# weiwei-ww/ML-VAE

Measured on AMD Instinct MI355X. Metric: spectrogram frames/sec + ELBO; 80-d log-mel B=256 at 1/2/4/8 MI355X, higher is better.
Workload: dtype bf16

## Files before the change

### ml-vae_amd/csrc/lstm_wide.hip

```cpp
#include "lstm_common.h"
#include <stdlib.h>
#include <type_traits>

namespace {

constexpr int WW = 8;
constexpr int FWD_KLF = 4;
template <int TPW> constexpr int bptt_groups() { return 2; }
#ifndef NT_AUX
#define NT_AUX 2
#endif

__device__ __forceinline__ void publish(__amdgpu_buffer_rsrc_t r, unsigned byte_off,
                                        unsigned long long v, bool plain) {
  if (plain) {
    u32x2 w = {(unsigned)v, (unsigned)(v >> 32)};
    __builtin_amdgcn_raw_buffer_store_b64(w, r, byte_off, 0, 0);
  } else {
    st_granule(r, byte_off, v);
  }
}

__device__ __forceinline__ int swz(int utt, int slot) { return slot ^ (utt & 15); }

template <int TPW, int NKC, int OCC, bool DBG = false, bool AS = false, bool ZP = false, int NT = 1,
          bool W12 = false>
__global__ __launch_bounds__(W12 ? 768 : 512, W12 ? 1 : OCC) void lstm_fwd_wide_kernel(LstmArgs a) {
  static_assert(NT == 1 || (NT == 2 && AS && TPW == 1), "two N-tiles: the asymmetric TPW-1 split");
  static_assert(!W12 || (AS && TPW == 1), "12 waves: the asymmetric TPW-1 split");
  constexpr int NWV = W12 ? 12 : 8;
  constexpr int NPOLL = W12 ? 8 : 4;
  constexpr int IO0 = NWV - 4;
  constexpr int BGW = BG * NT;
  constexpr int HJ = WW * TPW * 4;
  constexpr int H = NKC * 32;
  constexpr int PL = NKC / NPOLL;
  constexpr int ROWB = H * 2;
  constexpr int HIMG = BGW * ROWB;
  constexpr int GXU = 4 * HJ + 8;
  constexpr int OUB = 4 * HJ * 2 + 2 * HJ * 4 + 16;
  constexpr int NC8 = BGW * HJ / 8;
  constexpr int KLF = ((TPW == 1 && !AS) || W12) ? 0 : FWD_KLF;
  constexpr int KR = NKC - KLF;
  constexpr int HB = 4;
  constexpr int NQ = 16 * 4 * HJ / 4;
  constexpr int QPT = NQ / 256;
  static_assert(NQ % 256 == 0, "io split");
  extern __shared__ __attribute__((aligned(16))) char smem[];
  LSTAMP_DECL;
  RTS_DECL;
  char* himg = smem;
  unsigned short* gxr = reinterpret_cast<unsigned short*>(smem + 2 * HIMG);
  char* outr = reinterpret_cast<char*>(gxr + 2 * BGW * GXU);
  bf16x8* wlds = reinterpret_cast<bf16x8*>(outr + 2 * BGW * OUB);
  unsigned* dbl = reinterpret_cast<unsigned*>(wlds + 8 * TPW * KLF * 64);
  __shared__ int abort_flag;

  const int ngroups = 2 * a.NB, gstride = (ngroups + 7) & ~7;
  const int gid = blockIdx.x % gstride, js = blockIdx.x / gstride;
  if (gid >= ngroups) return;
  const int dir = gid / a.NB, grp = gid % a.NB;
  const int T = a.T, j0 = js * HJ;
  const int tid = threadIdx.x, lane = tid & 63;
  const int nlg = (DMODE(a) & (1 << 24)) ? 2 : 1, nmask = (1 << nlg) - 1;
  const int wave = __builtin_amdgcn_readfirstlane(tid >> 6);
  const float* W = dir ? a.W1 : a.W0;
  const int bi = lane & 15, q = lane >> 4;
  bool valid[NT];
#pragma unroll
  for (int n = 0; n < NT; ++n) valid[n] = grp * BGW + 16 * n + bi < a.B;

  static_assert(!AS || TPW == 1, "asymmetric split: TPW 1 only");
  constexpr int TPP = W12 ? 1 : AS ? 2 : TPW;
  constexpr int TPI = AS ? 0 : TPW;
  static_assert(NPOLL * TPP + 4 * TPI == WW * TPW, "every tile owned once");
  auto load_w = [&](auto* wreg, int m0, int mt) {
    for (int t = 0; t < mt; ++t) {
      const int m = m0 + t;
      const float* wrow = W + (size_t)((bi & 3) * H + j0 + 4 * m + (bi >> 2)) * H;
#pragma unroll
      for (int kc = 0; kc < NKC; ++kc) {
        const f32x4 w0 = *reinterpret_cast<const f32x4*>(wrow + kc * 32 + 8 * q);
        const f32x4 w1 = *reinterpret_cast<const f32x4*>(wrow + kc * 32 + 8 * q + 4);
        bf16x8 v;
#pragma unroll
        for (int e = 0; e < 4; ++e) { v[e] = f2bf(w0[e]); v[4 + e] = f2bf(w1[e]); }
        if (kc < KR) wreg[t][kc < KR ? kc : 0] = v;
        else wlds[(m * KLF + (kc - KR)) * 64 + lane] = v;
      }
    }
  };
  __shared__ int placement;
  const bool same_xcd = group_on_one_xcd(a.xtab + gid * a.NJ, a.NJ, js, &placement) &&
                        !(DMODE(a) & 32768);
  if (tid == 0) abort_flag = 0;

  const size_t xslot = (size_t)BGW * H;
  short* xb = reinterpret_cast<short*>(a.xbuf) + (size_t)(dir * a.NB + grp) * NSLOT * xslot;
  auto xr = make_rsrc(xb, (unsigned)(NSLOT * xslot * sizeof(short)));

  const int iot = tid - 64 * IO0;
  const bool io = wave >= IO0;
  const int iow = wave - IO0;
  typedef __attribute__((address_space(3))) void* lds_ptr_t;
  unsigned short* G16 = reinterpret_cast<unsigned short*>(a.G);
  const auto rgx = make_rsrc(G16 + (size_t)grp * BGW * T * 8 * H, 0xffffffffu);
  const bool tmaj = (DMODE(a) & 1024) != 0;
  auto rowof = [&](int b_, int t_) -> size_t { return tmaj ? (size_t)t_ * a.B + b_ : (size_t)b_ * T + t_; };
  const auto rgx_abs = make_rsrc(G16, (unsigned)min((size_t)a.B * T * 8 * H * 2, (size_t)0xffffffffu));
  unsigned short* zr = gxr;
  const auto rz = make_rsrc(a.Zb, (unsigned)min((size_t)a.B * T * a.ldz * 2, (size_t)0x7fffffff));
  auto io_load = [&](int s_) {
    if (s_ >= T || (s_ > 0 && (DMODE(a) & 8192))) return;
    const int t_ = dir ? T - 1 - s_ : s_;
    if constexpr (ZP) {
      if (iow < NT) {
        const int u = iow * 16 + (lane >> 2), b = grp * BGW + u;
        const unsigned off = b < a.B ? (unsigned)((((size_t)b * T + t_) * a.ldz + 8 * (lane & 3)) * 2) : 0x80000000u;
        __builtin_amdgcn_raw_ptr_buffer_load_lds(rz, (lds_ptr_t)(zr + ((s_ & 1) * BGW + iow * 16) * 32), 16,
                                                 off, 0, 0, NT_AUX);
      }
      return;
    }
    constexpr int UPW = BGW / 4;
#pragma unroll
    for (int i = 0; i < UPW; ++i) {
      const int u = iow * UPW + i, b = grp * BGW + u;
      if (b >= a.B) continue;
      const int g = lane / (HJ / 8), uu = (lane % (HJ / 8)) * 8;
      const unsigned off = tmaj ? (unsigned)((((size_t)t_ * a.B + b) * 8 * H + dir * 4 * H + g * H + j0 + uu) * 2)
                                : (unsigned)((((size_t)u * T + t_) * 8 * H + dir * 4 * H + g * H + j0 + uu) * 2);
      const auto rs = tmaj ? rgx_abs : rgx;
      unsigned short* dst = gxr + (s_ & 1) * BGW * GXU + u * GXU;
      if (lane < HJ / 2) __builtin_amdgcn_raw_ptr_buffer_load_lds(rs, (lds_ptr_t)dst, 16, off, 0, 0, NT_AUX);
    }
  };
  auto drop_bits = [&](int s_, int c8) -> unsigned {
    const int u = c8 / (HJ / 8), uu = (c8 % (HJ / 8)) * 8;
    const int t_ = dir ? T - 1 - s_ : s_;
    const size_t o = ((size_t)(grp * BGW + u) * T + t_) * 2 * H + dir * H + j0 + uu;
    const unsigned long long k = drop_key(a.dseed);
    const unsigned long long r0 = drop_quad(k, (a.doff + o) >> 2), r1 = drop_quad(k, (a.doff + o + 4) >> 2);
    unsigned bits = 0;
#pragma unroll
    for (int e = 0; e < 4; ++e) {
      bits |= (drop_elem_scale(r0, e, a.dkeep, 1.f) != 0.f ? 1u : 0u) << e;
      bits |= (drop_elem_scale(r1, e, a.dkeep, 1.f) != 0.f ? 1u : 0u) << (4 + e);
    }
    return bits;
  };
  auto io_store = [&](int s_) {
    if (s_ < 0 || s_ >= T || (DMODE(a) & 1)) return;
    const int t_ = dir ? T - 1 - s_ : s_;
    const char* src = outr + (s_ & 1) * BGW * OUB;
    constexpr int NG8 = BGW * 4 * HJ / 8;
    for (int ci = iot; ci < NG8; ci += 256) {
      const int row = ci / (HJ / 8), uu = (ci % (HJ / 8)) * 8;
      const int u = row >> 2, g = row & 3, b = grp * BGW + u;
      if (b >= a.B) continue;
      *reinterpret_cast<u32x4*>(G16 + rowof(b, t_) * 8 * H + dir * 4 * H + g * H + j0 + uu) =
          *reinterpret_cast<const u32x4*>(src + u * OUB + (g * HJ + uu) * 2);
    }
    constexpr int NQ2 = BGW * HJ / 4;
    for (int qi = iot; qi < NQ2; qi += 256) {
      const int u = qi / (HJ / 4), uu = (qi % (HJ / 4)) * 4, b = grp * BGW + u;
      if (b >= a.B) continue;
      const size_t o = rowof(b, t_) * 2 * H + dir * H + j0 + uu;
      const float* cf = reinterpret_cast<const float*>(src + u * OUB + 8 * HJ);
      *reinterpret_cast<f32x4*>(a.Cs + o) = *reinterpret_cast<const f32x4*>(cf + uu);
      if (a.Y) *reinterpret_cast<f32x4*>(a.Y + o) = *reinterpret_cast<const f32x4*>(cf + HJ + uu);
    }
    static_assert(2 * NC8 <= 256, "one h chunk per io thread");
    const bool drop8 = iot >= NC8;
    const int ci8 = drop8 ? iot - NC8 : iot;
    if (ci8 < NC8 && (drop8 ? (a.Ydb != nullptr || a.Y8 != nullptr) : a.Yb != nullptr)) {
      const int u = ci8 / (HJ / 8), uu = (ci8 % (HJ / 8)) * 8, b = grp * BGW + u;
      if (b < a.B) {
        const float* hf = reinterpret_cast<const float*>(src + u * OUB + 8 * HJ) + HJ;
        f32x4 v0 = *reinterpret_cast<const f32x4*>(hf + uu);
        f32x4 v1 = *reinterpret_cast<const f32x4*>(hf + uu + 4);
        size_t o = rowof(b, t_) * 2 * H + dir * H + j0 + uu;
        if (ZP && !drop8 && a.yb_prev) {
          if (s_ == 0)
            *reinterpret_cast<bf16x8*>(a.Yb + o) = bf16x8{0, 0, 0, 0, 0, 0, 0, 0};
          const int tn = dir ? t_ - 1 : t_ + 1;
          if (tn < 0 || tn >= T) return;
          o = rowof(b, tn) * 2 * H + dir * H + j0 + uu;
        }
        if (drop8) {
          const unsigned bits = dbl[(s_ & 1) * NC8 + ci8];
#pragma unroll
          for (int e = 0; e < 4; ++e) {
            v0[e] = (bits >> e) & 1 ? v0[e] * a.dscale : 0.f;
            v1[e] = (bits >> (4 + e)) & 1 ? v1[e] * a.dscale : 0.f;
          }
        }
        if (!drop8 || a.Ydb)
          *reinterpret_cast<bf16x8*>((drop8 ? a.Ydb : a.Yb) + o) =
              bf16x8{f2bf(v0[0]), f2bf(v0[1]), f2bf(v0[2]), f2bf(v0[3]),
                     f2bf(v1[0]), f2bf(v1[1]), f2bf(v1[2]), f2bf(v1[3])};
        if (drop8 && a.Y8) {
          const float xs = a.x8scale;
          *reinterpret_cast<u32x2*>(a.Y8 + o) =
              u32x2{pack4_fp8(v0[0] * xs, v0[1] * xs, v0[2] * xs, v0[3] * xs),
                    pack4_fp8(v1[0] * xs, v1[1] * xs, v1[2] * xs, v1[3] * xs)};
        }
      }
    }
  };
  const bool want_drop = a.Ydb || a.Y8;
  const bool late_bits = want_drop && !(DMODE(a) & (1 << 27));
  const bool late_dma_s = (2 * a.NB * a.NJ <= 64) != ((DMODE(a) & (1 << 17)) != 0);
  auto run = [&](auto io_tag) {
    constexpr bool IO = decltype(io_tag)::value;
    constexpr int MT = IO ? TPI : TPP;
    constexpr int MTA = MT > 0 ? MT : 1;
    const int m0 = IO ? NPOLL * TPP + iow * TPI : wave * TPP;
    bf16x8 wreg[MTA][KR];
    load_w(wreg, m0, MT);
    bf16x8 wz[ZP ? MTA : 1];
    f32x4 bz4[ZP ? MTA : 1];
    if constexpr (ZP) {
      const float* Wz = dir ? a.Wz1 : a.Wz0;
      const float* bih = a.bz[2 * dir];
      const float* bhh = a.bz[2 * dir + 1];
#pragma unroll
      for (int t = 0; t < MT; ++t) {
        const int m = m0 + t;
        const float* wrow = Wz + (size_t)((bi & 3) * H + j0 + 4 * m + (bi >> 2)) * 32 + 8 * q;
        const f32x4 w0 = *reinterpret_cast<const f32x4*>(wrow);
        const f32x4 w1 = *reinterpret_cast<const f32x4*>(wrow + 4);
#pragma unroll
        for (int e = 0; e < 4; ++e) { wz[t][e] = f2bf(w0[e]); wz[t][4 + e] = f2bf(w1[e]); }
#pragma unroll
        for (int g4 = 0; g4 < 4; ++g4) bz4[t][g4] = bih[g4 * H + j0 + 4 * m + q] + bhh[g4 * H + j0 + 4 * m + q];
      }
    }
    constexpr bool PURE_IO = IO && MT == 0;
    if (IO) {
      io_load(0);
      io_load(1);
      asm volatile("s_waitcnt vmcnt(0)" ::: "memory");
    }
    __syncthreads();
    float c[MTA][NT];
#pragma unroll
    for (int t = 0; t < MTA; ++t)
#pragma unroll
      for (int n = 0; n < NT; ++n) c[t][n] = 0.f;
    stagger_start(gid, DMODE(a));
    for (int s = 0; s < T; ++s) {
      LSTAMP(0);
      IOSTAMP(0);
      f32x4 acc[MTA][NT];
#pragma unroll
      for (int t = 0; t < MTA; ++t)
#pragma unroll
        for (int n = 0; n < NT; ++n) acc[t][n] = f32x4{0.f, 0.f, 0.f, 0.f};
      char* hb = himg + (s & 1) * HIMG;
      float gxv[MTA][NT][4];
      unsigned short gxh[MTA][NT][4];
      auto read_gx = [&]() {
        if constexpr (ZP) {
          if constexpr (MT > 0) {
#pragma unroll
            for (int n = 0; n < NT; ++n) {
              const bf16x8 zf = *reinterpret_cast<const bf16x8*>(zr + ((s & 1) * BGW + 16 * n + bi) * 32 + 8 * q);
#pragma unroll
              for (int t = 0; t < MT; ++t) {
                const f32x4 r = __builtin_amdgcn_mfma_f32_16x16x32_bf16(wz[t], zf, bz4[t], 0, 0, 0);
#pragma unroll
                for (int g4 = 0; g4 < 4; ++g4) gxv[t][n][g4] = r[g4];
              }
            }
          }
          return;
        }
#pragma unroll
        for (int n = 0; n < NT; ++n) {
          const unsigned short* gx = gxr + ((s & 1) * BGW + 16 * n + bi) * GXU;
#pragma unroll
          for (int t = 0; t < MT; ++t) {
            const int u = 4 * (m0 + t) + q;
#pragma unroll
            for (int g4 = 0; g4 < 4; ++g4) gxh[t][n][g4] = gx[g4 * HJ + u];
          }
        }
      };
      if (s == 0) read_gx();
      if (s > 0) {
        if (IO) {
          if (!(DMODE(a) & 16384))
            asm volatile("s_waitcnt vmcnt(0)" ::: "memory");
          IOSTAMP(1);
        } else {
          const unsigned tag = step_tag_lg(s - 1, nlg);
          const unsigned xbase = (unsigned)(((s - 1) & nmask) * xslot) + (((wave * PL * 32 + 8 * q) >> 3) * BGW + bi) * 8;
          auto poll_off = [&](int i) -> unsigned {
            return xbase + (unsigned)((i / NT) * (32 / 8) * BGW + (i % NT) * 16) * 8;
          };
          constexpr int PLN = PL * NT;
          u32x4 hv[PLN];
          unsigned spins = 0;
          const bool partial = (int)gridDim.x >= 256 && !(DMODE(a) & (1 << 28));
#pragma unroll
          for (int i = 0; i < PLN; ++i) hv[i] = u32x4{tag ^ 1u, 0u, tag ^ 1u, 0u};
          while (true) {
#pragma unroll
            for (int i = 0; i < PLN; ++i)
              if (!partial || !tags_ok(hv[i], tag, true, true)) hv[i] = ld_sc1_b128(xr, poll_off(i) * sizeof(short));
            if (late_bits && spins == 0 && tid < NC8) dbl[((s - 1) & 1) * NC8 + tid] = drop_bits(s - 1, tid);
            bool ok = true;
#pragma unroll
            for (int i = 0; i < PLN; ++i) ok &= tags_ok(hv[i], tag, true, true);
            if (__all(ok)) break;
            if (++spins > SPIN_LIMIT) {
              if (lane == 0) { atomicExch(a.err, 1); abort_flag = 1; }
              break;
            }
            if (partial && (DMODE(a) & (1 << 30))) __builtin_amdgcn_s_sleep(1);
            else if (partial || (DMODE(a) & 262144)) __builtin_amdgcn_s_sleep(2);
            else __builtin_amdgcn_s_sleep(6);
          }
          LSTAMP(1);
          RTS(8 + wave);
#pragma unroll
          for (int i = 0; i < PLN; ++i)
            *reinterpret_cast<u32x4*>(hb + (16 * (i % NT) + bi) * ROWB + swz(bi, (wave * PL + i / NT) * 4 + q) * 16) = hv[i];
        }
        if (wave < 8) LWSTAMP();
        __syncthreads();
        LSTAMP(2);
        if (abort_flag) break;
        IOSTAMP(2);
        if (IO && (PURE_IO || !late_dma_s)) io_load(s + 1);
        if (PURE_IO && s > 0) io_store(s - 1);
        IOSTAMP(3);
        if constexpr (!ZP || MT == 0) read_gx();
        const bool first = AS ? !IO : IO ? !(DMODE(a) & (1 << 25)) : (DMODE(a) & (1 << 26)) != 0;
        if (first) __builtin_amdgcn_s_setprio(1);
        constexpr int KLA = KLF > 0 ? KLF : 1;
        bf16x8 wl[MTA][KLA];
        bf16x8 zf[NT];
#pragma unroll
        for (int k0 = 0; k0 < NKC; k0 += HB) {
          bf16x8 hfrag[HB][NT];
#pragma unroll
          for (int i = 0; i < HB; ++i)
#pragma unroll
            for (int n = 0; n < NT; ++n)
              hfrag[i][n] = *reinterpret_cast<const bf16x8*>(hb + (16 * n + bi) * ROWB + swz(bi, ((k0 + i + KR) % NKC) * 4 + q) * 16);
          if (k0 == 0) {
#pragma unroll
            for (int t = 0; t < MT; ++t)
#pragma unroll
              for (int j = 0; j < KLF; ++j) wl[t][j] = wlds[((m0 + t) * KLF + j) * 64 + lane];
            if constexpr (ZP) {
#pragma unroll
              for (int n = 0; n < NT; ++n)
                zf[n] = *reinterpret_cast<const bf16x8*>(zr + ((s & 1) * BGW + 16 * n + bi) * 32 + 8 * q);
            }
          }
          __builtin_amdgcn_sched_barrier(0);
          if constexpr (ZP) {
            if (k0 == 0) {
#pragma unroll
              for (int t = 0; t < MT; ++t)
#pragma unroll
                for (int n = 0; n < NT; ++n) {
                  const f32x4 r = __builtin_amdgcn_mfma_f32_16x16x32_bf16(wz[t], zf[n], bz4[t], 0, 0, 0);
#pragma unroll
                  for (int g4 = 0; g4 < 4; ++g4) gxv[t][n][g4] = r[g4];
                }
            }
          }
#pragma unroll
          for (int i = 0; i < HB; ++i) {
            const int kc = (k0 + i + KR) % NKC;
#pragma unroll
            for (int t = 0; t < MT; ++t) {
              const bf16x8 wf = kc < KR ? wreg[t][kc < KR ? kc : 0] : wl[t][kc >= KR ? kc - KR : 0];
#pragma unroll
              for (int n = 0; n < NT; ++n)
                acc[t][n] = __builtin_amdgcn_mfma_f32_16x16x32_bf16(wf, hfrag[i][n], acc[t][n], 0, 0, 0);
            }
          }
        }
        __builtin_amdgcn_sched_barrier(0);
        if (MT > 0) asm volatile("s_nop 7\n\ts_nop 7" ::: "memory");
        __builtin_amdgcn_sched_barrier(0);
        if (first) __builtin_amdgcn_s_setprio(0);
        LSTAMP(3);
        IOSTAMP(4);
      }
      float hvals[MTA][NT], gates[MTA][NT][4];
#pragma unroll
      for (int n = 0; n < NT; ++n)
#pragma unroll
        for (int t = 0; t < MT; ++t) {
          float gi[4];
#pragma unroll
          for (int g4 = 0; g4 < 4; ++g4) gi[g4] = ZP ? gxv[t][n][g4] : h2f(gxh[t][n][g4]);
          const float ig = sigmoid_fast(acc[t][n][0] + gi[0]);
          const float fg = sigmoid_fast(acc[t][n][1] + gi[1]);
          const float gg = tanh_fast(acc[t][n][2] + gi[2]);
          const float og = sigmoid_fast(acc[t][n][3] + gi[3]);
          c[t][n] = valid[n] ? fg * c[t][n] + ig * gg : 0.f;
          hvals[t][n] = valid[n] ? og * tanh_fast(c[t][n]) : 0.f;
          gates[t][n][0] = ig; gates[t][n][1] = fg; gates[t][n][2] = gg; gates[t][n][3] = og;
        }
      if (DBG && !(DMODE(a) & (1 << 23))) {
        __builtin_amdgcn_sched_barrier(0);
        LSTAMP(5);
        __builtin_amdgcn_sched_barrier(0);
      }
      if (s + 1 < T) {
        const unsigned tag = step_tag_lg(s, nlg);
        unsigned long long gr[MTA][NT];
#pragma unroll
        for (int n = 0; n < NT; ++n)
#pragma unroll
          for (int t = 0; t < MT; ++t) {
            const unsigned hu = __float_as_uint(hvals[t][n]);
            const unsigned x1 = __builtin_amdgcn_permlane16_swap(hu, hu, false, false)[1];
            const unsigned x2 = __builtin_amdgcn_permlane32_swap(hu, hu, false, false)[1];
            const unsigned x3 = __builtin_amdgcn_permlane32_swap(x1, x1, false, false)[1];
            const float h1 = __uint_as_float(x1), h2 = __uint_as_float(x2), h3 = __uint_as_float(x3);
            gr[t][n] = pack_bf16(hvals[t][n], h1, h2, h3, tag);
          }
        if (AS && q == 0) {
          if constexpr (MT == 2) {
            const int u0 = j0 + 4 * m0;
#pragma unroll
            for (int n = 0; n < NT; ++n) {
              const u32x4 v = {(unsigned)gr[0][n], (unsigned)(gr[0][n] >> 32), (unsigned)gr[1][n], (unsigned)(gr[1][n] >> 32)};
              const unsigned cell = (unsigned)((s & nmask) * xslot) + ((u0 >> 3) * BGW + 16 * n + bi) * 8 + (u0 & 7);
              if (same_xcd) __builtin_amdgcn_raw_buffer_store_b128(v, xr, cell * sizeof(short), 0, 0);
              else st_sc1_b128(xr, cell * sizeof(short), v);
            }
          } else {
#pragma unroll
            for (int n = 0; n < NT; ++n)
#pragma unroll
              for (int t = 0; t < MT; ++t) {
                const int u0 = j0 + 4 * (m0 + t);
                publish(xr, ((unsigned)((s & nmask) * xslot) + ((u0 >> 3) * BGW + 16 * n + bi) * 8 + (u0 & 7)) * sizeof(short),
                        gr[t][n], same_xcd);
              }
          }
        } else if (q == 0) {
          const int u0 = j0 + 4 * TPW * wave;
          const unsigned cell = (unsigned)((s & nmask) * xslot) + ((u0 >> 3) * 16 + bi) * 8 + (u0 & 7);
          if constexpr (TPW == 2) {
            const u32x4 v = {(unsigned)gr[0][0], (unsigned)(gr[0][0] >> 32), (unsigned)gr[1][0], (unsigned)(gr[1][0] >> 32)};
            if (same_xcd) __builtin_amdgcn_raw_buffer_store_b128(v, xr, cell * sizeof(short), 0, 0);
            else st_sc1_b128(xr, cell * sizeof(short), v);
          } else {
            publish(xr, cell * sizeof(short), gr[0][0], same_xcd);
          }
        }
      }
      LSTAMP(4);
      RTS(wave);
      IOSTAMP(5);
      if (!IO && (DMODE(a) & (1 << 23))) {
        asm volatile("s_waitcnt vmcnt(0)" ::: "memory");
        LSTAMP(5);
      }
      if (IO && !PURE_IO && late_dma_s) io_load(s + 1);
      if (IO && !PURE_IO && s > 0) io_store(s - 1);
      IOSTAMP(6);
#pragma unroll
      for (int n = 0; n < NT; ++n) {
        char* ob = outr + ((s & 1) * BGW + 16 * n + bi) * OUB;
        unsigned short* og = reinterpret_cast<unsigned short*>(ob);
        float* of = reinterpret_cast<float*>(ob + 8 * HJ);
#pragma unroll
        for (int t = 0; t < MT; ++t) {
          const int u = 4 * (m0 + t) + q;
          og[u] = f2h(gates[t][n][0]); og[HJ + u] = f2h(gates[t][n][1]);
          og[2 * HJ + u] = f2h(gates[t][n][2]); og[3 * HJ + u] = f2h(gates[t][n][3]);
          of[u] = c[t][n]; of[HJ + u] = hvals[t][n];
        }
      }
      LSTAMP(6);
      if (!IO && want_drop && tid < NC8 && (!late_bits || s + 1 == T)) dbl[(s & 1) * NC8 + tid] = drop_bits(s, tid);
      LSTAMP(7);
    }
    __syncthreads();
    if (IO) io_store(T - 1);
  };
  if (io) run(std::true_type{});
  else run(std::false_type{});
  LSTAMP_FLUSH();
  RTS_FLUSH();
}

template <int TPW, int NKC, int OCC, bool F8 = false, bool DYB = false, bool DBG = false>
__global__ __launch_bounds__(512, OCC) void lstm_bwd_wide_kernel(LstmArgs a) {
  constexpr int HJ = 32 * TPW;
  constexpr int H = NKC * 32;
  constexpr int NJ = H / HJ;
  constexpr int NTW = NKC / 4;
  constexpr int KC = 4 * HJ / 32;
  constexpr int KLB = TPW == 1 ? 0 : KC / 4;
  constexpr int KR = KC - KLB;
  constexpr int BKB = TPW == 1 ? 4 : 1;
  constexpr int ROWB = 4 * HJ * 2;
  constexpr int AIMG = 16 * ROWB;
  constexpr int NPL = NJ / 8;
  constexpr int CPG = 2 * HJ / 64;
  static_assert(NPL >= 1 && CPG >= 1 && NPL * CPG == 2, "two 16-byte partial loads per lane");
  extern __shared__ __attribute__((aligned(16))) char smem[];
  LSTAMP_DECL;
  RTS_DECL;
  char* aimg = smem;
  bf16x8* wlds = reinterpret_cast<bf16x8*>(smem + 2 * AIMG);
  constexpr int CG_B = 4 * HJ * 2 + 16;
  constexpr int CF_B = HJ * 4 + 32;
  constexpr int CD_B = DYB ? HJ * 2 + 32 : CF_B;
  static_assert(((CG_B + CF_B + CD_B) / 4) % 8 == 4 || ((CG_B + CF_B + CD_B) / 4) % 64 == 20,
                "conflict-free staged rows");
  constexpr int CUTT = CG_B + CF_B + CD_B;
  char* cst = smem + 2 * AIMG + (size_t)8 * NTW * KLB * 64 * 16;
  __shared__ int abort_flag;

  const int ngroups = 2 * a.NB, gstride = (ngroups + 7) & ~7;
  const int gid = blockIdx.x % gstride, js = blockIdx.x / gstride;
  if (gid >= ngroups) return;
  const int dir = gid / a.NB, grp = gid % a.NB;
  const int T = a.T, j0 = js * HJ;
  const int tid = threadIdx.x, lane = tid & 63;
  const int nlg = (DMODE(a) & (1 << 24)) ? 2 : 1, nmask = (1 << nlg) - 1;
  const int wave = __builtin_amdgcn_readfirstlane(tid >> 6);
  const float* W = dir ? a.W1 : a.W0;
  const int bi = lane & 15, q = lane >> 4;

  bf16x8 wreg[NTW][KR];
  static_assert(KLB > 0 || KR == KC, "");
#pragma unroll
  for (int nt = 0; nt < NTW; ++nt) {
    const int n = (wave * NTW + nt) * 16 + bi;
#pragma unroll
    for (int kc = 0; kc < KC; ++kc) {
      bf16x8 v;
#pragma unroll
      for (int e = 0; e < 8; ++e) {
        const int k = kc * 32 + 8 * q + e;
        v[e] = f2bf(W[(size_t)((k / HJ) * H + j0 + (k % HJ)) * H + n]);
      }
      if (kc < KR) wreg[nt][kc < KR ? kc : 0] = v;
      else wlds[((wave * NTW + nt) * KLB + (kc - KR)) * 64 + lane] = v;
    }
  }
  __shared__ int placement;
  const bool same_xcd = group_on_one_xcd(a.xtab + gid * NJ, NJ, js, &placement) &&
                        !(DMODE(a) & 32768);
  if (tid == 0) abort_flag = 0;
  if (DBG && DPTR(a) && (DMODE(a) & 8) && tid == 0) a.dbg[blockIdx.x] = same_xcd ? 1 : 2;
  __syncthreads();

  const size_t xslot = (size_t)NJ * NJ * HJ * 16;
  short* xb = reinterpret_cast<short*>(a.xbuf) + (size_t)(dir * a.NB + grp) * NSLOT * xslot;
  auto xr = make_rsrc(xb, (unsigned)(NSLOT * xslot * sizeof(short)));

  auto rs_perm = [](int g) { return g ^ ((g & 4) ? 3 : 0); };
  const int arow = rs_perm(js / NPL);
  const int gq = tid >> 3, pg = lane & 7;
  int uc[CPG], cu[CPG];
  bool bv[CPG];
#pragma unroll
  for (int ci = 0; ci < CPG; ++ci) {
    const int cb = gq * CPG + ci;
    uc[ci] = cb >> 1;
    cu[ci] = (cb & 1) * 8 + rs_perm(pg);
    bv[ci] = grp * BG + cu[ci] < a.B;
  }
  constexpr int NGC = 16 * 4 * HJ / 8, NFC = 16 * HJ / 4, NDC = DYB ? 16 * HJ / 8 : NFC;
  constexpr int NCH = NGC + NFC + NDC;
  constexpr int CPT = (NCH + 511) / 512;
  static_assert(DYB || NCH % 512 == 0, "whole chunks per thread");
  static_assert(NGC % 64 == 0 && NFC % 64 == 0 && NDC % 64 == 0, "chunk kinds change at whole waves");
  const size_t gbase = (size_t)grp * BG * T;
  const auto rG = make_rsrc(reinterpret_cast<const unsigned short*>(a.G) + gbase * 8 * H, 0xffffffffu);
  const auto rC = make_rsrc(a.Cs + gbase * 2 * H, 0xffffffffu);
  const auto rY = DYB ? make_rsrc(a.dYb + gbase * 2 * H, 0xffffffffu) : make_rsrc(a.Y + gbase * 2 * H, 0xffffffffu);
  u32x4 creg[CPT];
  auto chunk_lds = [&](int c) -> int {
    if (c < NGC) {
      const int u = c / (4 * HJ / 8), k = c % (4 * HJ / 8);
      return u * CUTT + k * 16;
    }
    const int f = c - NGC;
    if (f < NFC) {
      const int u = f / (HJ / 4), k = f % (HJ / 4);
      return u * CUTT + CG_B + k * 16;
    }
    const int r = f - NFC, upr = DYB ? HJ / 8 : HJ / 4;
    return (r / upr) * CUTT + CG_B + CF_B + (r % upr) * 16;
  };
  const int ulast = a.B - 1 - grp * BG;
  auto load_cell = [&](int s_) {
    const int sc = s_ < T ? s_ : T - 1;
    const int t_ = dir ? sc : T - 1 - sc;
    const int tp_ = dir ? t_ + 1 : t_ - 1;
    const int tpc = tp_ < 0 ? 0 : (tp_ >= T ? T - 1 : tp_);
#pragma unroll
    for (int i = 0; i < CPT; ++i) {
      const int cw0 = wave * 64 + 512 * i;
      const int cw = cw0 < NCH ? cw0 : 0;
      const int c = cw + lane;
      const bool isg = cw < NGC, ydy = cw - NGC >= NFC;
      const int r = c - NGC - (ydy ? NFC : 0);
      const int ug = c / (4 * HJ / 8), k = c % (4 * HJ / 8), g = k / (HJ / 8), ugu = (k % (HJ / 8)) * 8;
      const int upr = (ydy && DYB) ? HJ / 8 : HJ / 4, epr = (ydy && DYB) ? 8 : 4;
      const int uf = r / upr, ufu = (r % upr) * epr;
      const int u = min(isg ? ug : uf, ulast);
      const unsigned og = ((unsigned)(u * T + t_) * 8 * H + dir * 4 * H + g * H + j0 + ugu) * 2u;
      const unsigned of = ((unsigned)(u * T + (ydy ? t_ : tpc)) * 2 * H + dir * H + j0 + ufu) *
                          ((ydy && DYB) ? 2u : 4u);
      creg[i] = __builtin_bit_cast(
          u32x4, __builtin_amdgcn_raw_buffer_load_b128(isg ? rG : (ydy ? rY : rC), isg ? og : of, 0, NT_AUX));
    }
  };
  auto stage_cell = [&](int s_) {
    char* dst = cst + (s_ & 1) * 16 * CUTT;
#pragma unroll
    for (int i = 0; i < CPT; ++i) {
      if (wave * 64 + 512 * i < NCH)
        *reinterpret_cast<u32x4*>(dst + chunk_lds(wave * 64 + 512 * i + lane)) = creg[i];
    }
  };
  float dc[CPG], cc[CPG], bsum[CPG][4];
#pragma unroll
  for (int ci = 0; ci < CPG; ++ci) {
    dc[ci] = 0.f;
    cc[ci] = 0.f;
    bsum[ci][0] = bsum[ci][1] = bsum[ci][2] = bsum[ci][3] = 0.f;
    if (bv[ci]) {
      const int t0 = dir ? 0 : T - 1;
      cc[ci] = a.Cs[((size_t)(grp * BG + cu[ci]) * T + t0) * 2 * H + dir * H + j0 + uc[ci]];
    }
  }
#pragma unroll
  for (int i = 0; i < CPT; ++i) creg[i] = u32x4{0u, 0u, 0u, 0u};
  load_cell(0);
  stage_cell(0);
  load_cell(1);
  __syncthreads();
  float g8max = 0.f;
  const float g8s = (F8 && a.dG8) ? *a.g8scale : 0.f;

  auto step = [&](int s) -> bool {
    LSTAMP(0);
    float xi[CPG], xf[CPG], xgg[CPG], xo[CPG], xcp[CPG], xdy[CPG];
#pragma unroll
    for (int ci = 0; ci < CPG; ++ci) {
      const char* cu_row = cst + (s & 1) * 16 * CUTT + cu[ci] * CUTT;
      const unsigned short* xg = reinterpret_cast<const unsigned short*>(cu_row) + uc[ci];
      xi[ci] = h2f(xg[0]); xf[ci] = h2f(xg[HJ]); xgg[ci] = h2f(xg[2 * HJ]); xo[ci] = h2f(xg[3 * HJ]);
      xcp[ci] = reinterpret_cast<const float*>(cu_row + CG_B)[uc[ci]];
      if constexpr (DYB)
        xdy[ci] = __uint_as_float((unsigned)reinterpret_cast<const unsigned short*>(cu_row + CG_B + CF_B)[uc[ci]] << 16);
      else
        xdy[ci] = reinterpret_cast<const float*>(cu_row + CG_B + CF_B)[uc[ci]];
    }
    float dh[CPG];
#pragma unroll
    for (int ci = 0; ci < CPG; ++ci) dh[ci] = 0.f;
    float fA[CPG], fF[CPG], f0[CPG], f1[CPG], f2[CPG], f3[CPG];
    auto factors = [&]() {
#pragma unroll
      for (int ci = 0; ci < CPG; ++ci) {
        const float cpv = s + 1 < T ? xcp[ci] : 0.f;
        const float tc = tanh_fast(cc[ci]);
        const bool v = bv[ci];
        fA[ci] = v ? xo[ci] * (1.f - tc * tc) : 0.f;
        fF[ci] = v ? xf[ci] : 0.f;
        f0[ci] = v ? xgg[ci] * xi[ci] * (1.f - xi[ci]) : 0.f;
        f1[ci] = v ? cpv * xf[ci] * (1.f - xf[ci]) : 0.f;
        f2[ci] = v ? xi[ci] * (1.f - xgg[ci] * xgg[ci]) : 0.f;
        f3[ci] = v ? tc * xo[ci] * (1.f - xo[ci]) : 0.f;
        cc[ci] = xcp[ci];
      }
    };
    u32x4 pv[CPG][NPL];
    const bool early_stage = !(DMODE(a) & (1 << 19)) && s > 0;
    if (s > 0) {
      const unsigned tag = step_tag_lg(s - 1, nlg);
      const size_t sb = (size_t)((s - 1) & nmask) * xslot + (size_t)js * NJ * HJ * 16;
      unsigned spins = 0;
      auto sweep = [&]() {
#pragma unroll
        for (int ci = 0; ci < CPG; ++ci)
#pragma unroll
          for (int i = 0; i < NPL; ++i) {
            const int p = pg * NPL + i;
            const size_t off = sb + ((size_t)p * HJ + uc[ci]) * 16 + (cu[ci] >> 3) * 8;
            pv[ci][i] = ld_sc1_b128(xr, (unsigned)(off * sizeof(short)));
          }
      };
      sweep();
      factors();
      if (early_stage) stage_cell(s + 1);
      while (true) {
        bool ok = true;
#pragma unroll
        for (int ci = 0; ci < CPG; ++ci)
#pragma unroll
          for (int i = 0; i < NPL; ++i) ok &= tags_ok(pv[ci][i], tag, true, true);
        if (__all(ok)) break;
        if (++spins > SPIN_LIMIT) {
          if (lane == 0) { atomicExch(a.err, 1); abort_flag = 1; }
          break;
        }
        if (DMODE(a) & 262144) __builtin_amdgcn_s_sleep(2);
        else __builtin_amdgcn_s_sleep(1);
        sweep();
      }
    } else {
      factors();
    }
    LSTAMP(1);
    if (!(DMODE(a) & (3 << 21))) LWSTAMP();
    RTS(8 + wave);
    if (!early_stage) stage_cell(s + 1);
    LSTAMP(5);
    const bool late_pf = (int)gridDim.x >= 256 && !(DMODE(a) & (1 << 16));
    if (!late_pf) load_cell(s + 2);
    LSTAMP(6);
    if (s > 0) {
#pragma unroll
      for (int ci = 0; ci < CPG; ++ci) {
        float v[8];
#pragma unroll
        for (int d = 0; d < 4; ++d) {
          v[2 * d] = __uint_as_float(pv[ci][0][d] << 16);
          v[2 * d + 1] = __uint_as_float(pv[ci][0][d] & 0xffff0000u);
        }
#pragma unroll
        for (int i = 1; i < NPL; ++i)
#pragma unroll
          for (int d = 0; d < 4; ++d) {
            v[2 * d] += __uint_as_float(pv[ci][i][d] << 16);
            v[2 * d + 1] += __uint_as_float(pv[ci][i][d] & 0xffff0000u);
          }
        float w4[4], w2[2];
#pragma unroll
        for (int k = 0; k < 4; ++k) w4[k] = v[k] + dpp_f<0x141>(v[k + 4]);
#pragma unroll
        for (int k = 0; k < 2; ++k) w2[k] = w4[k] + dpp_f<0x4E>(w4[k + 2]);
        dh[ci] = w2[0] + dpp_f<0xB1>(w2[1]);
      }
    }
    LSTAMP(2);
    if (DMODE(a) & (1 << 21)) LWSTAMP();
    char* ab = aimg + (s & 1) * AIMG;
#pragma unroll
    for (int ci = 0; ci < CPG; ++ci) {
      const float dht = xdy[ci] + dh[ci];
      const float dcs = __builtin_fmaf(dht, fA[ci], dc[ci]);
      dc[ci] = dcs * fF[ci];
      const float dg[4] = {dcs * f0[ci], dcs * f1[ci], dcs * f2[ci], dht * f3[ci]};
      const int u = uc[ci], r = cu[ci] ^ arow;
#pragma unroll
      for (int g = 0; g < 4; ++g) {
        const int k = g * HJ + u;
        *reinterpret_cast<short*>(ab + r * ROWB + swz(r, k >> 3) * 16 + (k & 7) * 2) = f2bf(dg[g]);
      }
#pragma unroll
      for (int g = 0; g < 4; ++g) bsum[ci][g] += dg[g];
    }
    if (DMODE(a) & (1 << 22)) LWSTAMP();
    __syncthreads();
    LSTAMP(7);
    if (late_pf) load_cell(s + 2);
    LSTAMP(3);
    if (abort_flag) return false;
    if (s + 1 < T) {
      const unsigned tag = step_tag_lg(s, nlg);
      const size_t sb = (size_t)(s & nmask) * xslot;
      constexpr int NGRP = bptt_groups<TPW>();
      static_assert(NTW % NGRP == 0 && (TPW != 1 || (NTW / NGRP) % 2 == 0), "tile groups");
      constexpr int TPH = NTW / NGRP;
      constexpr bool AONCE = BKB == KC && NGRP > 1;
      bf16x8 afr_all[AONCE ? KC : 1];
      if constexpr (AONCE) {
#pragma unroll
        for (int i = 0; i < KC; ++i)
          afr_all[i] = *reinterpret_cast<const bf16x8*>(ab + bi * ROWB + swz(bi, i * 4 + q) * 16);
        __builtin_amdgcn_sched_barrier(0);
      }
#pragma unroll
      for (int hf = 0; hf < NGRP; ++hf) {
        f32x4 acc[TPH];
#pragma unroll
        for (int t = 0; t < TPH; ++t) acc[t] = f32x4{0.f, 0.f, 0.f, 0.f};
#pragma unroll
        for (int k0 = 0; k0 < KC; k0 += BKB) {
          bf16x8 afr[BKB];
          if constexpr (AONCE) {
#pragma unroll
            for (int i = 0; i < BKB; ++i) afr[i] = afr_all[k0 + i];
          } else {
#pragma unroll
            for (int i = 0; i < BKB; ++i)
              afr[i] = *reinterpret_cast<const bf16x8*>(ab + bi * ROWB + swz(bi, (k0 + i) * 4 + q) * 16);
            __builtin_amdgcn_sched_barrier(0);
          }
#pragma unroll
          for (int i = 0; i < BKB; ++i) {
            const int kc = k0 + i;
#pragma unroll
            for (int t = 0; t < TPH; ++t) {
              const int nt = hf * TPH + t;
              const bf16x8 wf = kc < KR ? wreg[nt][kc < KR ? kc : 0] : wlds[((wave * NTW + nt) * KLB + (kc - KR)) * 64 + lane];
              acc[t] = __builtin_amdgcn_mfma_f32_16x16x32_bf16(afr[i], wf, acc[t], 0, 0, 0);
            }
          }
        }
        if constexpr (TPW != 1) {
#pragma unroll
          for (int t = 0; t < TPH; ++t) {
            const int n = (wave * NTW + hf * TPH + t) * 16 + bi;
            const int cons = n / HJ, un = n % HJ;
            const size_t off = sb + (((size_t)cons * NJ + js) * HJ + un) * 16 + 4 * q;
            publish(xr, (unsigned)(off * sizeof(short)),
                    pack_bf16(acc[t][0], acc[t][1], acc[t][2], acc[t][3], tag), same_xcd);
          }
        } else {
#pragma unroll
          for (int pr = 0; pr < TPH / 2; ++pr) {
            const int ta = 2 * pr, tb = 2 * pr + 1;
            const unsigned long long ga = pack_bf16(acc[ta][0], acc[ta][1], acc[ta][2], acc[ta][3], tag);
            const unsigned long long gb = pack_bf16(acc[tb][0], acc[tb][1], acc[tb][2], acc[tb][3], tag);
            const auto lo = __builtin_amdgcn_permlane16_swap((unsigned)ga, (unsigned)gb, false, false);
            const auto hi = __builtin_amdgcn_permlane16_swap((unsigned)(ga >> 32), (unsigned)(gb >> 32), false, false);
            const u32x4 v = {lo[0], hi[0], lo[1], hi[1]};
            const int n = (wave * NTW + hf * TPH + ((q & 1) ? tb : ta)) * 16 + bi;
            const int cons = n / HJ, un = n % HJ;
            const size_t off = sb + (((size_t)cons * NJ + js) * HJ + un) * 16 + 8 * (q >> 1);
            if (same_xcd) __builtin_amdgcn_raw_buffer_store_b128(v, xr, (unsigned)(off * sizeof(short)), 0, 0);
            else st_sc1_b128(xr, (unsigned)(off * sizeof(short)), v);
          }
        }
      }
    }
    LSTAMP(4);
    RTS(wave);
    if (!(DMODE(a) & 1)) {
      constexpr int NSL = 16 * 4 * HJ / 8;
      const int t = dir ? s : T - 1 - s;
      for (int sl = tid; sl < NSL; sl += 512) {
        const int r = sl / (4 * HJ / 8), kslot = sl % (4 * HJ / 8);
        const int b = grp * BG + (r ^ arow);
        if (b >= a.B) continue;
        const int k = kslot * 8, g = k / HJ, u = k % HJ;
        const u32x4 v = *reinterpret_cast<const u32x4*>(ab + r * ROWB + swz(r, kslot) * 16);
        const size_t o = ((size_t)b * T + t) * 8 * H + dir * 4 * H + g * H + j0 + u;
        if (!F8 || a.dGb) *reinterpret_cast<u32x4*>(a.dGb + o) = v;
        if constexpr (F8) {
          float f[8];
#pragma unroll
          for (int e = 0; e < 4; ++e) {
            f[2 * e] = __uint_as_float(v[e] << 16);
            f[2 * e + 1] = __uint_as_float(v[e] & 0xffff0000u);
          }
#pragma unroll
          for (int e = 0; e < 8; ++e) g8max = fmaxf(g8max, fabsf(f[e]));
          if (a.dG8)
            *reinterpret_cast<u32x2*>(a.dG8 + o) =
                u32x2{pack4_fp8(f[0] * g8s, f[1] * g8s, f[2] * g8s, f[3] * g8s),
                      pack4_fp8(f[4] * g8s, f[5] * g8s, f[6] * g8s, f[7] * g8s)};
        }
      }
    }
    return true;
  };
  stagger_start(gid, DMODE(a));
  for (int s = 0; s < T; ++s)
    if (!step(s)) break;
  LSTAMP_FLUSH();
  RTS_FLUSH();
  if constexpr (F8) {
    float m = g8max;
#pragma unroll
    for (int o = 32; o > 0; o >>= 1) m = fmaxf(m, __shfl_xor(m, o, 64));
    if (lane == 0) atomicMax(a.g8amax, __float_as_uint(m));
  }
  if (a.dbias) {
    float bs[4];
#pragma unroll
    for (int g = 0; g < 4; ++g) {
      float v = bsum[0][g];
#pragma unroll
      for (int ci = 1; ci < CPG; ++ci) v += bsum[ci][g];
      v += __shfl_xor(v, 1, 64);
      v += __shfl_xor(v, 2, 64);
      v += __shfl_xor(v, 4, 64);
      if (CPG == 1) v += __shfl_xor(v, 8, 64);
      bs[g] = v;
    }
    if (pg == 0 && (CPG == 2 || (gq & 1) == 0)) {
#pragma unroll
      for (int g = 0; g < 4; ++g)
        a.dbias[(size_t)grp * 8 * H + dir * 4 * H + g * H + j0 + uc[0]] = bs[g];
    }
  }
}

struct WidePlan {
  int tpw, nkc, NB, NJ, HJ;
  int nt;
  bool w12;
  size_t lds, xbytes, xtab_off;
  bool ok;
};

int wide_cus() {
  int dev = 0, cus = 256;
  if (hipGetDevice(&dev) != hipSuccess ||
      hipDeviceGetAttribute(&cus, hipDeviceAttributeMultiprocessorCount, dev) != hipSuccess)
    cus = 256;
  return cus;
}

size_t wide_lds(int H, int hj, bool fwd, int nt = 1) {
  const size_t bgw = (size_t)BG * nt;
  if (fwd)
    return 2 * bgw * H * 2 + 2 * bgw * (4 * hj + 8) * 2 +
           2 * bgw * (4 * hj * 2 + 2 * hj * 4 + 16) +
           (size_t)8 * (hj / 32) * FWD_KLF * 64 * 16 +
           2 * (bgw * hj / 8) * 4;
  return (size_t)2 * 16 * 4 * hj * 2 +
         (size_t)8 * (H / 128) * (hj == 32 ? 0 : hj / 32) * 64 * 16 +
         (size_t)2 * 16 * ((4 * hj * 2 + 16) + 2 * (hj * 4 + 32));
}

WidePlan wide_plan(int B, int H, bool fwd, int mode = 0) {
  WidePlan p{};
  p.ok = false;
  p.nt = 1;
  p.w12 = false;
  if (H != 512) return p;
  p.nkc = H / 32;
  p.NB = (B + BG - 1) / BG;
  const int cus = wide_cus();
  if (fwd && (mode & 512) && 2 * p.NB * (H / 32) > cus) {
    const int nb2 = (B + 2 * BG - 1) / (2 * BG);
    if (2 * nb2 * (H / 32) <= cus) {
      p.nt = 2; p.tpw = 1; p.HJ = 32; p.NJ = H / 32; p.NB = nb2; p.ok = true;
    }
  }
  if (!p.ok)
  for (int tpw = 1; tpw <= 2; ++tpw) {
    if (fwd && tpw * p.nkc * 4 > 128) break;
    p.NB = (B + BG - 1) / BG;
    const int hj = 32 * tpw, nj = H / hj;
    if (!fwd && (nj < 8 || nj % 8)) continue;
    if (2 * p.NB * nj <= cus) {
      p.tpw = tpw; p.HJ = hj; p.NJ = nj; p.ok = true;
      break;
    }
  }
  if (!p.ok) return p;
  if (fwd && p.tpw == 1) p.w12 = !(mode & 2048);
  p.lds = wide_lds(H, p.HJ, fwd, p.nt);
  if (fwd) p.xbytes = (size_t)2 * p.NB * NSLOT * BG * p.nt * H * 2;
  else p.xbytes = (size_t)2 * p.NB * NSLOT * p.NJ * p.NJ * p.HJ * 16 * 2;
  if (p.lds < (size_t)MIN_LDS) p.lds = MIN_LDS;
  p.xtab_off = p.xbytes;
  p.xbytes += (size_t)2 * p.NB * p.NJ * sizeof(unsigned);
  return p;
}

template <int TPW, int NKC, int OCC>
int launch_wide(bool fwd, const LstmArgs& a, const WidePlan& p, hipStream_t s) {
  const bool dbg = a.dbg != nullptr;
  constexpr bool AS1 = TPW == 1;
  const bool zp = a.Zb != nullptr;
  auto k = (fwd && p.w12)
               ? (p.nt == 2 ? (dbg ? lstm_fwd_wide_kernel<1, NKC, OCC, true, true, false, 2, true>
                                   : zp ? lstm_fwd_wide_kernel<1, NKC, OCC, false, true, true, 2, true>
                                        : lstm_fwd_wide_kernel<1, NKC, OCC, false, true, false, 2, true>)
                            : (dbg ? lstm_fwd_wide_kernel<1, NKC, OCC, true, true, false, 1, true>
                                   : zp ? lstm_fwd_wide_kernel<1, NKC, OCC, false, true, true, 1, true>
                                        : lstm_fwd_wide_kernel<1, NKC, OCC, false, true, false, 1, true>))
         : (fwd && p.nt == 2)
               ? (dbg ? lstm_fwd_wide_kernel<1, NKC, OCC, true, true, false, 2>
                      : zp ? lstm_fwd_wide_kernel<1, NKC, OCC, false, true, true, 2>
                           : lstm_fwd_wide_kernel<1, NKC, OCC, false, true, false, 2>)
         : fwd ? (dbg ? lstm_fwd_wide_kernel<TPW, NKC, OCC, true, AS1>
                      : zp ? lstm_fwd_wide_kernel<TPW, NKC, OCC, false, AS1, true>
                           : lstm_fwd_wide_kernel<TPW, NKC, OCC, false, AS1>)
               : (a.g8amax ? (a.dYb ? lstm_bwd_wide_kernel<TPW, NKC, OCC, true, true>
                                    : lstm_bwd_wide_kernel<TPW, NKC, OCC, true, false>)
                           : (a.dYb ? (dbg ? lstm_bwd_wide_kernel<TPW, NKC, OCC, false, true, true>
                                           : lstm_bwd_wide_kernel<TPW, NKC, OCC, false, true>)
                                    : (dbg ? lstm_bwd_wide_kernel<TPW, NKC, OCC, false, false, true>
                                           : lstm_bwd_wide_kernel<TPW, NKC, OCC, false>)));
  if (hipFuncSetAttribute((const void*)k, hipFuncAttributeMaxDynamicSharedMemorySize, (int)p.lds) != hipSuccess) {
    mlvae_set_error("lstm_wide: cannot reserve %zu B LDS", p.lds);
    return 2;
  }
  k<<<dim3(((2 * p.NB + 7) & ~7) * p.NJ), (fwd && p.w12) ? 768 : 512, p.lds, s>>>(a);
  MLVAE_CHECK_LAUNCH();
  return 0;
}

}

bool lstm_wide_t_ok(int T, int H) {
  return (size_t)2 * BG * T * 8 * H * 2 <= 0xffffffffull && (size_t)2 * BG * T * 2 * H * 4 <= 0xffffffffull;
}

int lstm_wide_workgroups(int B, int H, bool fwd) {
  WidePlan p = wide_plan(B, H, fwd);
  if (!p.ok) return 0;
  return 2 * p.NB * p.NJ;
}

size_t lstm_wide_xbytes(int B, int H, bool fwd) {
  WidePlan p = wide_plan(B, H, fwd), q = wide_plan(B, H, fwd, 512);
  if (!p.ok) return 0;
  return p.xbytes > q.xbytes ? p.xbytes : q.xbytes;
}

int lstm_wide_run(bool fwd, int B, int T, int H, const float* W0, const float* W1, float* G,
                  float* Cs, float* Y, void* xbuf, size_t xbytes, int* err, hipStream_t st,
                  unsigned short* yb, unsigned short* dgb, float* dbias, unsigned short* ydb,
                  unsigned long long dseed, unsigned long long doff, float dp,
                  unsigned long long* dbg, int dbg_mode, const WideFp8& f8, const unsigned short* dyb,
                  const WideZ& wz) {
  WidePlan p = wide_plan(B, H, fwd, dbg_mode);
  if (!p.ok) return -1;
  if (!lstm_wide_t_ok(T, H)) {
    mlvae_set_error("lstm_wide: T=%d too long for the wide kernels' 32-bit batch-group addressing at H=%d "
                    "(mlvae_lstm_gates_fp16_t(B, T, H, prec) = 0: pass fp32 gates)", T, H);
    return 1;
  }
  if (!xbuf || xbytes < p.xbytes || !err) {
    mlvae_set_error("lstm_wide: exchange workspace too small (need %zu B)", p.xbytes);
    return 1;
  }
  LstmArgs a{};
  a.ndir = 2;
  a.B = B; a.T = T; a.H = H; a.NB = p.NB; a.NJ = p.NJ; a.HJ = p.HJ; a.Kp = H; a.K4p = 4 * H;
  a.W0 = W0; a.W1 = W1; a.G = G; a.Cs = Cs; a.Y = Y; a.xbuf = xbuf; a.err = err;
  a.dbg = dbg; a.dbg_mode = dbg_mode; a.xcd_local = 0; a.Yb = yb; a.dGb = dgb;
  a.dbias = dbias; a.Ydb = ydb; a.dseed = dseed; a.doff = doff; a.dkeep = 1.f - dp;
  a.Y8 = f8.y8; a.x8scale = f8.x8scale; a.dG8 = f8.dg8; a.g8scale = f8.g8scale; a.g8amax = f8.g8amax;
  a.dYb = fwd ? nullptr : dyb;
  if (wz.zb && dbg) a.dbg = dbg = nullptr;
  if (wz.zb) {
    if (!fwd || !wz.w0 || !wz.w1 || !wz.b[0] || !wz.b[1] || !wz.b[2] || !wz.b[3] ||
        wz.ldz < 32 || wz.ldz % 8 || ((uintptr_t)wz.zb % 16)) {
      mlvae_set_error("lstm_wide: the fused z projection needs the forward, "
                      "both W_ih and all four biases, a 16-byte aligned z with ldz >= 32, ldz %% 8 == 0");
      return 1;
    }
    a.Zb = wz.zb; a.ldz = wz.ldz; a.Wz0 = wz.w0; a.Wz1 = wz.w1; a.yb_prev = wz.yb_prev;
    for (int i = 0; i < 4; ++i) a.bz[i] = wz.b[i];
  }
  if (a.Y8 && (!fwd || !(a.x8scale > 0.f) || !(dp >= 0.f && dp < 1.f))) {
    mlvae_set_error("lstm_wide: the e4m3 dropout(h) output needs the forward, a positive scale and 0 <= p < 1");
    return 1;
  }
  if (a.dG8 && (!a.g8scale || !a.g8amax)) {
    mlvae_set_error("lstm_wide: the fp8 dG copy needs its scale and amax words");
    return 1;
  }
  a.dscale = dp < 1.f ? 1.f / (1.f - dp) : 0.f;
  a.xtab = reinterpret_cast<unsigned*>(static_cast<char*>(xbuf) + p.xtab_off);
  if (hipMemsetAsync(xbuf, 0, p.xbytes, st) != hipSuccess) {
    mlvae_set_error("lstm_wide: memset failed");
    return 2;
  }
  return p.tpw == 2 ? launch_wide<2, 16, 2>(fwd, a, p, st) : launch_wide<1, 16, 2>(fwd, a, p, st);
}
```

Before: 13.46 million.

## Extend 12-wave forward LSTM kernel to TPW-2 with LDS-staged weights

Enables the 12-wave forward variant (tile-less io waves) for the TPW=2 configuration, which previously used only 8 waves. To fit register budget at 768 threads, z-projection weights and biases move to LDS and are interleaved into the recurrent MFMA k-loop in smaller batches (HB=2), with LDS weight chunks loaded per batch and precomputed swizzled h offsets. This aims to raise wave count and overlap io with compute, at the cost of extra LDS traffic per step and a larger LDS footprint.

```diff
diff --git a/ml-vae_amd/csrc/lstm_wide.hip b/ml-vae_amd/csrc/lstm_wide.hip
--- a/ml-vae_amd/csrc/lstm_wide.hip
+++ b/ml-vae_amd/csrc/lstm_wide.hip
@@ -27,7 +27,9 @@
           bool W12 = false>
 __global__ __launch_bounds__(W12 ? 768 : 512, W12 ? 1 : OCC) void lstm_fwd_wide_kernel(LstmArgs a) {
   static_assert(NT == 1 || (NT == 2 && AS && TPW == 1), "two N-tiles: the asymmetric TPW-1 split");
-  static_assert(!W12 || (AS && TPW == 1), "12 waves: the asymmetric TPW-1 split");
+  static_assert(!W12 || AS, "12 waves: tile-less io waves");
+  static_assert(!W12 || TPW == 1 || NT == 1, "12 waves at TPW 2: one N-tile");
+  constexpr bool W2 = W12 && TPW == 2;
   constexpr int NWV = W12 ? 12 : 8;
   constexpr int NPOLL = W12 ? 8 : 4;
   constexpr int IO0 = NWV - 4;
@@ -40,9 +42,9 @@
   constexpr int GXU = 4 * HJ + 8;
   constexpr int OUB = 4 * HJ * 2 + 2 * HJ * 4 + 16;
   constexpr int NC8 = BGW * HJ / 8;
-  constexpr int KLF = ((TPW == 1 && !AS) || W12) ? 0 : FWD_KLF;
+  constexpr int KLF = ((TPW == 1 && !AS) || (W12 && TPW == 1)) ? 0 : FWD_KLF;
   constexpr int KR = NKC - KLF;
-  constexpr int HB = 4;
+  constexpr int HB = W2 ? 2 : 4;
   constexpr int NQ = 16 * 4 * HJ / 4;
   constexpr int QPT = NQ / 256;
   static_assert(NQ % 256 == 0, "io split");
@@ -51,7 +53,8 @@
   RTS_DECL;
   char* himg = smem;
   unsigned short* gxr = reinterpret_cast<unsigned short*>(smem + 2 * HIMG);
-  char* outr = reinterpret_cast<char*>(gxr + 2 * BGW * GXU);
+  constexpr int GXB = (W2 && ZP) ? 2 * BGW * 32 * 2 + WW * TPW * (4 * 16 + 64 * 16) : 2 * BGW * GXU * 2;
+  char* outr = reinterpret_cast<char*>(gxr) + GXB;
   bf16x8* wlds = reinterpret_cast<bf16x8*>(outr + 2 * BGW * OUB);
   unsigned* dbl = reinterpret_cast<unsigned*>(wlds + 8 * TPW * KLF * 64);
   __shared__ int abort_flag;
@@ -70,8 +73,8 @@
 #pragma unroll
   for (int n = 0; n < NT; ++n) valid[n] = grp * BGW + 16 * n + bi < a.B;
 
-  static_assert(!AS || TPW == 1, "asymmetric split: TPW 1 only");
-  constexpr int TPP = W12 ? 1 : AS ? 2 : TPW;
+  static_assert(!AS || TPW == 1 || W12, "asymmetric split in 8 waves: TPW 1 only");
+  constexpr int TPP = W12 ? TPW : AS ? 2 : TPW;
   constexpr int TPI = AS ? 0 : TPW;
   static_assert(NPOLL * TPP + 4 * TPI == WW * TPW, "every tile owned once");
   auto load_w = [&](auto* wreg, int m0, int mt) {
@@ -87,6 +90,10 @@
         for (int e = 0; e < 4; ++e) { v[e] = f2bf(w0[e]); v[4 + e] = f2bf(w1[e]); }
         if (kc < KR) wreg[t][kc < KR ? kc : 0] = v;
         else wlds[(m * KLF + (kc - KR)) * 64 + lane] = v;
+        if constexpr (W2) {
+          if (kc < KR) asm volatile("" : "+v"(wreg[t][kc < KR ? kc : 0]));
+          if (kc % 8 == 7) __builtin_amdgcn_sched_barrier(0);
+        }
       }
     }
   };
@@ -109,6 +116,8 @@
   auto rowof = [&](int b_, int t_) -> size_t { return tmaj ? (size_t)t_ * a.B + b_ : (size_t)b_ * T + t_; };
   const auto rgx_abs = make_rsrc(G16, (unsigned)min((size_t)a.B * T * 8 * H * 2, (size_t)0xffffffffu));
   unsigned short* zr = gxr;
+  f32x4* bzl = reinterpret_cast<f32x4*>(zr + 2 * BGW * 32);
+  bf16x8* wzl = reinterpret_cast<bf16x8*>(bzl + WW * TPW * 4);
   const auto rz = make_rsrc(a.Zb, (unsigned)min((size_t)a.B * T * a.ldz * 2, (size_t)0x7fffffff));
   auto io_load = [&](int s_) {
     if (s_ >= T || (s_ > 0 && (DMODE(a) & 8192))) return;
@@ -234,6 +243,10 @@
         for (int e = 0; e < 4; ++e) { wz[t][e] = f2bf(w0[e]); wz[t][4 + e] = f2bf(w1[e]); }
 #pragma unroll
         for (int g4 = 0; g4 < 4; ++g4) bz4[t][g4] = bih[g4 * H + j0 + 4 * m + q] + bhh[g4 * H + j0 + 4 * m + q];
+        if constexpr (W2) {
+          wzl[m * 64 + lane] = wz[t];
+          if (bi == 0) bzl[4 * m + q] = bz4[t];
+        }
       }
     }
     constexpr bool PURE_IO = IO && MT == 0;
@@ -248,6 +261,9 @@
     for (int t = 0; t < MTA; ++t)
 #pragma unroll
       for (int n = 0; n < NT; ++n) c[t][n] = 0.f;
+    int hsw[4];
+#pragma unroll
+    for (int j = 0; j < 4; ++j) hsw[j] = bi * ROWB + swz(bi, 4 * j + q) * 16;
     stagger_start(gid, DMODE(a));
     for (int s = 0; s < T; ++s) {
       LSTAMP(0);
@@ -268,7 +284,11 @@
               const bf16x8 zf = *reinterpret_cast<const bf16x8*>(zr + ((s & 1) * BGW + 16 * n + bi) * 32 + 8 * q);
 #pragma unroll
               for (int t = 0; t < MT; ++t) {
-                const f32x4 r = __builtin_amdgcn_mfma_f32_16x16x32_bf16(wz[t], zf, bz4[t], 0, 0, 0);
+                f32x4 r;
+                if constexpr (W2)
+                  r = __builtin_amdgcn_mfma_f32_16x16x32_bf16(wzl[(m0 + t) * 64 + lane], zf, bzl[4 * (m0 + t) + q], 0, 0, 0);
+                else
+                  r = __builtin_amdgcn_mfma_f32_16x16x32_bf16(wz[t], zf, bz4[t], 0, 0, 0);
 #pragma unroll
                 for (int g4 = 0; g4 < 4; ++g4) gxv[t][n][g4] = r[g4];
               }
@@ -340,17 +360,41 @@
         const bool first = AS ? !IO : IO ? !(DMODE(a) & (1 << 25)) : (DMODE(a) & (1 << 26)) != 0;
         if (first) __builtin_amdgcn_s_setprio(1);
         constexpr int KLA = KLF > 0 ? KLF : 1;
-        bf16x8 wl[MTA][KLA];
+        bf16x8 wl[MTA][W2 ? HB : KLA];
         bf16x8 zf[NT];
+        f32x4 bzf;
+        bf16x8 wzf;
+        constexpr int ZK0 = KLF;
 #pragma unroll
         for (int k0 = 0; k0 < NKC; k0 += HB) {
           bf16x8 hfrag[HB][NT];
 #pragma unroll
           for (int i = 0; i < HB; ++i)
 #pragma unroll
-            for (int n = 0; n < NT; ++n)
-              hfrag[i][n] = *reinterpret_cast<const bf16x8*>(hb + (16 * n + bi) * ROWB + swz(bi, ((k0 + i + KR) % NKC) * 4 + q) * 16);
-          if (k0 == 0) {
+            for (int n = 0; n < NT; ++n) {
+              const int kc = (k0 + i + KR) % NKC;
+              if constexpr (W2)
+                hfrag[i][n] = *reinterpret_cast<const bf16x8*>(hb + hsw[kc & 3] + (kc >> 2) * 256);
+              else
+                hfrag[i][n] = *reinterpret_cast<const bf16x8*>(hb + (16 * n + bi) * ROWB + swz(bi, kc * 4 + q) * 16);
+            }
+          if constexpr (W2) {
+            static_assert(!W2 || KLF % HB == 0, "a batch is all LDS chunks or all register chunks");
+            if (k0 < KLF) {
+#pragma unroll
+              for (int t = 0; t < MT; ++t)
+#pragma unroll
+                for (int i = 0; i < HB; ++i) wl[t][i] = wlds[((m0 + t) * KLF + k0 + i) * 64 + lane];
+            }
+            if constexpr (ZP) {
+              if (k0 >= ZK0 && k0 < ZK0 + MT * HB) {
+                const int t = (k0 - ZK0) / HB;
+                zf[0] = *reinterpret_cast<const bf16x8*>(zr + ((s & 1) * BGW + bi) * 32 + 8 * q);
+                bzf = bzl[4 * (m0 + t) + q];
+                wzf = wzl[(m0 + t) * 64 + lane];
+              }
+            }
+          } else if (k0 == 0) {
 #pragma unroll
             for (int t = 0; t < MT; ++t)
 #pragma unroll
@@ -362,7 +406,13 @@
             }
           }
           __builtin_amdgcn_sched_barrier(0);
-          if constexpr (ZP) {
+          if constexpr (ZP && W2) {
+            if (k0 >= ZK0 && k0 < ZK0 + MT * HB) {
+              const f32x4 r = __builtin_amdgcn_mfma_f32_16x16x32_bf16(wzf, zf[0], bzf, 0, 0, 0);
+#pragma unroll
+              for (int g4 = 0; g4 < 4; ++g4) gxv[(k0 - ZK0) / HB][0][g4] = r[g4];
+            }
+          } else if constexpr (ZP) {
             if (k0 == 0) {
 #pragma unroll
               for (int t = 0; t < MT; ++t)
@@ -379,7 +429,7 @@
             const int kc = (k0 + i + KR) % NKC;
 #pragma unroll
             for (int t = 0; t < MT; ++t) {
-              const bf16x8 wf = kc < KR ? wreg[t][kc < KR ? kc : 0] : wl[t][kc >= KR ? kc - KR : 0];
+              const bf16x8 wf = kc < KR ? wreg[t][kc < KR ? kc : 0] : wl[t][W2 ? i : kc >= KR ? kc - KR : 0];
 #pragma unroll
               for (int n = 0; n < NT; ++n)
                 acc[t][n] = __builtin_amdgcn_mfma_f32_16x16x32_bf16(wf, hfrag[i][n], acc[t][n], 0, 0, 0);
@@ -451,7 +501,7 @@
         } else if (q == 0) {
           const int u0 = j0 + 4 * TPW * wave;
           const unsigned cell = (unsigned)((s & nmask) * xslot) + ((u0 >> 3) * 16 + bi) * 8 + (u0 & 7);
-          if constexpr (TPW == 2) {
+          if constexpr (TPW == 2 && !AS) {
             const u32x4 v = {(unsigned)gr[0][0], (unsigned)(gr[0][0] >> 32), (unsigned)gr[1][0], (unsigned)(gr[1][0] >> 32)};
             if (same_xcd) __builtin_amdgcn_raw_buffer_store_b128(v, xr, cell * sizeof(short), 0, 0);
             else st_sc1_b128(xr, cell * sizeof(short), v);
@@ -925,10 +975,12 @@
   return cus;
 }
 
-size_t wide_lds(int H, int hj, bool fwd, int nt = 1) {
+size_t wide_lds(int H, int hj, bool fwd, int nt = 1, bool zp2 = false) {
   const size_t bgw = (size_t)BG * nt;
   if (fwd)
-    return 2 * bgw * H * 2 + 2 * bgw * (4 * hj + 8) * 2 +
+    return 2 * bgw * H * 2 +
+           (zp2 ? 2 * bgw * 32 * 2 + (size_t)8 * (hj / 32) * (4 * 16 + 64 * 16)
+                : 2 * bgw * (4 * hj + 8) * 2) +
            2 * bgw * (4 * hj * 2 + 2 * hj * 4 + 16) +
            (size_t)8 * (hj / 32) * FWD_KLF * 64 * 16 +
            2 * (bgw * hj / 8) * 4;
@@ -937,7 +989,7 @@
          (size_t)2 * 16 * ((4 * hj * 2 + 16) + 2 * (hj * 4 + 32));
 }
 
-WidePlan wide_plan(int B, int H, bool fwd, int mode = 0) {
+WidePlan wide_plan(int B, int H, bool fwd, int mode = 0, bool zp = false) {
   WidePlan p{};
   p.ok = false;
   p.nt = 1;
@@ -964,8 +1016,8 @@
     }
   }
   if (!p.ok) return p;
-  if (fwd && p.tpw == 1) p.w12 = !(mode & 2048);
-  p.lds = wide_lds(H, p.HJ, fwd, p.nt);
+  if (fwd) p.w12 = !(mode & 2048);
+  p.lds = wide_lds(H, p.HJ, fwd, p.nt, zp && p.w12 && p.tpw == 2);
   if (fwd) p.xbytes = (size_t)2 * p.NB * NSLOT * BG * p.nt * H * 2;
   else p.xbytes = (size_t)2 * p.NB * NSLOT * p.NJ * p.NJ * p.HJ * 16 * 2;
   if (p.lds < (size_t)MIN_LDS) p.lds = MIN_LDS;
@@ -983,9 +1035,9 @@
                ? (p.nt == 2 ? (dbg ? lstm_fwd_wide_kernel<1, NKC, OCC, true, true, false, 2, true>
                                    : zp ? lstm_fwd_wide_kernel<1, NKC, OCC, false, true, true, 2, true>
                                         : lstm_fwd_wide_kernel<1, NKC, OCC, false, true, false, 2, true>)
-                            : (dbg ? lstm_fwd_wide_kernel<1, NKC, OCC, true, true, false, 1, true>
-                                   : zp ? lstm_fwd_wide_kernel<1, NKC, OCC, false, true, true, 1, true>
-                                        : lstm_fwd_wide_kernel<1, NKC, OCC, false, true, false, 1, true>))
+                            : (dbg ? lstm_fwd_wide_kernel<TPW, NKC, OCC, true, true, false, 1, true>
+                                   : zp ? lstm_fwd_wide_kernel<TPW, NKC, OCC, false, true, true, 1, true>
+                                        : lstm_fwd_wide_kernel<TPW, NKC, OCC, false, true, false, 1, true>))
          : (fwd && p.nt == 2)
                ? (dbg ? lstm_fwd_wide_kernel<1, NKC, OCC, true, true, false, 2>
                       : zp ? lstm_fwd_wide_kernel<1, NKC, OCC, false, true, true, 2>
@@ -1032,7 +1084,7 @@
                   unsigned long long dseed, unsigned long long doff, float dp,
                   unsigned long long* dbg, int dbg_mode, const WideFp8& f8, const unsigned short* dyb,
                   const WideZ& wz) {
-  WidePlan p = wide_plan(B, H, fwd, dbg_mode);
+  WidePlan p = wide_plan(B, H, fwd, dbg_mode, fwd && wz.zb != nullptr);
   if (!p.ok) return -1;
   if (!lstm_wide_t_ok(T, H)) {
     mlvae_set_error("lstm_wide: T=%d too long for the wide kernels' 32-bit batch-group addressing at H=%d "
```

New measurement: 13.64 million, median of 6. 1.01x the previous value.
